# mmaker/c-lwe-snarks

Hardware: AMD Instinct MI355X
Metric: snark_proofs_per_sec (higher is better)
Workload: dtype u32 limbs (704-bit integers mod 2^704) + AES-256 bytes; int8 digits on the matrix cores, int32 accumulation (exact)

## Files before the change

c-lwe-snarks_amd/__init__.py:

```python
from __future__ import annotations

import ctypes
import os
from dataclasses import dataclass

import numpy as np

_HERE = os.path.dirname(os.path.abspath(__file__))
LIB_PATH = os.environ.get("MFHIP_LIB") or os.path.join(_HERE, "libmfhip.so")
P = 0xFFFFFFFB


class MfhError(RuntimeError):
    pass


@dataclass(frozen=True)
class Params:

    n: int = 1470
    logq: int = 736
    d: int = 1 << 15
    m: int = 21845

# ... 40 lines not shown

DEBUG = Params(d=256, m=64)
DEFAULT = Params()


class _CParams(ctypes.Structure):
    _fields_ = [("n", ctypes.c_uint32), ("logq", ctypes.c_uint32), ("d", ctypes.c_uint32), ("m", ctypes.c_uint32)]


_lib = None

EXPORTS = [
    "mfh_ctx_create", "mfh_ctx_destroy", "mfh_set_stream", "mfh_sync", "mfh_scrub_staging", "mfh_last_error", "mfh_set_seed",
    "mfh_keystream", "mfh_sample_rows", "mfh_ct_add", "mfh_ct_mul_ui", "mfh_ct_addmul_ui", "mfh_eval_rows",
    "mfh_encrypt_rows", "mfh_decrypt", "mfh_ct_smudge", "mfh_ssp_upload", "mfh_witness_poly", "mfh_version",
    "mfh_workspace_bytes", "mfh_last_kernel_ms", "mfh_set_timing", "mfh_set_overlap", "mfh_eval_rows_multi", "mfh_prove_batch", "mfh_crs_mm_image_bytes", "mfh_crs_expand_mm", "mfh_crs_set_resident_mm", "mfh_witness_poly_multi", "mfh_witness_poly_mm", "mfh_poly_h_multi", "mfh_poly_mul", "mfh_poly_add", "mfh_poly_prepare_t",
    "mfh_ssp_prepare", "mfh_poly_h", "mfh_setup_messages", "mfh_setup", "mfh_setup_image", "mfh_crs_image_set_b", "mfh_prove",
    "mfh_prove_partial", "mfh_prove_finish", "mfh_ct_to_lanes", "mfh_ct_from_lanes", "mfh_lanes_per_value", "mfh_digest128", "mfh_timing_drain", "mfh_timing_busy_ms", "mfh_timing_work_rows", "mfh_set_batch_image", "mfh_set_batch_slabs", "mfh_set_expand_path", "mfh_set_encrypt_path", "mfh_set_batch_launch", "mfh_set_batch_bw", "mfh_set_mm_chunk_rows", "mfh_set_mm_pack", "mfh_set_poly_exact", "mfh_poly_exact_fallbacks", "mfh_poly_exact_points", "mfh_set_poly_exact_points", "mfh_set_mm_stream", "mfh_add_dotp", "mfh_set_encrypt_chunks", "mfh_set_witness_per", "mfh_set_eval_path", "mfh_set_decrypt_path", "mfh_decrypt_rows",
    "mfh_crs_mm_share_bytes", "mfh_crs_expand_mm_share", "mfh_crs_set_resident_mm_share", "mfh_batch_chain", "mfh_batch_witness_cols", "mfh_batch_chain_from_w", "mfh_witness_poly_mm_cols", "mfh_prove_batch_partial", "mfh_prove_batch_finish",
    "mfh_resident_row_bytes", "mfh_crs_expand", "mfh_eval_rows_resident", "mfh_crs_set_resident",
    "mfh_witness_lanes", "mfh_witness_from_lanes", "mfh_prove_partial_w", "mfh_verify",
    "mfh_ssp_set_prg", "mfh_ssp_prg_make_t", "mfh_ssp_prg_fill",
    "mfh_resident_share_rows", "mfh_crs_expand_share", "mfh_crs_set_resident_share", "mfh_crs_set_resident_prefix",
    "mfh_prove_batch_supergroup", "mfh_prove_batch_stream_wait", "mfh_set_mm_width",
    "mfh_setup_public", "mfh_prove_public", "mfh_prove_batch_public", "mfh_vk_derive", "mfh_verify_public",
    "mfh_ssp_from_rows", "mfh_ssp_set_rows", "mfh_ssp_rows_fill", "mfh_ssp_rows_violations", "mfh_circuit_create", "mfh_circuit_destroy", "mfh_circuit_assign",
    "mfh_circuit_create_global", "mfh_circuit_create_ex", "mfh_circuit_create_out", "mfh_circuit_create_sum",
    "mfh_merkle_create", "mfh_merkle_destroy", "mfh_merkle_set_leaves", "mfh_merkle_root", "mfh_merkle_nodes", "mfh_merkle_paths",
    "mfh_sha256_records", "mfh_merkle_set_records", "mfh_merkle_update_rows", "mfh_merkle_update_records",
    "mfh_merkle_absent_rows", "mfh_merkle_insert_keys", "mfh_merkle_update_rows_cut", "mfh_merkle_update_records_cut", "mfh_merkle_insert_keys_cut",
    "mfh_merkle_remove_keys", "mfh_merkle_remove_keys_cut", "mfh_merkle_transfer_keys", "mfh_merkle_transfer_keys_cut",
    "mfh_merkle_paths_cut", "mfh_merkle_absent_rows_cut", "mfh_merkle_range_rows", "mfh_merkle_range_rows_cut",
]


def load_library():
    global _lib
    if _lib is not None:
        return _lib
    if not os.path.exists(LIB_PATH):
        raise MfhError(f"{LIB_PATH} is missing: run `python -c 'import __graft_entry__ as g; g.build()'` "
                       "(hipcc --offload-arch=gfx950).  There is no CPU fallback.")
    lib = ctypes.CDLL(LIB_PATH)
    vp, u64, sz, i32, u32 = ctypes.c_void_p, ctypes.c_uint64, ctypes.c_size_t, ctypes.c_int, ctypes.c_uint32
    sig = {
        "mfh_ctx_create": (i32, [ctypes.POINTER(vp), i32, ctypes.POINTER(_CParams)]),
        "mfh_ctx_destroy": (None, [vp]),
        "mfh_set_stream": (i32, [vp, vp]),
        "mfh_sync": (i32, [vp]),
        "mfh_scrub_staging": (i32, [vp]),
        "mfh_last_error": (ctypes.c_char_p, [vp]),
        "mfh_set_seed": (i32, [vp, ctypes.c_char_p]),
        "mfh_keystream": (i32, [vp, u64, vp, sz]),
        "mfh_sample_rows": (i32, [vp, u64, sz, vp]),
        "mfh_ct_add": (i32, [vp, vp, vp, vp, sz]),
        "mfh_ct_mul_ui": (i32, [vp, vp, vp, u32, sz]),
        "mfh_ct_addmul_ui": (i32, [vp, vp, vp, u32, sz]),
        "mfh_eval_rows": (i32, [vp, u64, sz, vp, vp, vp, vp, vp, i32]),
        "mfh_encrypt_rows": (i32, [vp, u64, sz, vp, vp, vp, vp]),
        "mfh_decrypt": (i32, [vp, vp, vp, sz, vp]),
        "mfh_ct_smudge": (i32, [vp, vp, sz, ctypes.c_char_p, sz, ctypes.c_char_p]),
        "mfh_ssp_upload": (i32, [vp, vp, vp, sz, sz]),
        "mfh_witness_poly": (i32, [vp, vp, ctypes.c_char_p, u32, vp]),
        "mfh_version": (ctypes.c_char_p, []),
        "mfh_workspace_bytes": (sz, [vp]),
        "mfh_last_kernel_ms": (ctypes.c_float, [vp, ctypes.c_char_p]),
        "mfh_set_timing": (i32, [vp, i32]),
        "mfh_set_overlap": (i32, [vp, i32]),
        "mfh_eval_rows_multi": (i32, [vp, u64, sz, vp, vp, u32, u32, vp, i32]),
        "mfh_poly_h_multi": (i32, [vp, vp, vp, u32]),
        "mfh_witness_poly_mm": (i32, [vp, vp, u32, ctypes.c_char_p, sz, vp, vp]),
        "mfh_witness_poly_multi": (i32, [vp, vp, u32, ctypes.c_char_p, sz, vp, vp]),
        "mfh_crs_mm_image_bytes": (sz, [vp]),
        "mfh_crs_expand_mm": (i32, [vp, vp, vp]),
        "mfh_crs_set_resident_mm": (i32, [vp, vp]),
        "mfh_prove_batch": (i32, [vp, vp, vp, u32, ctypes.c_char_p, sz, vp, ctypes.c_char_p, sz, ctypes.c_char_p, vp]),
        "mfh_prove_batch_supergroup": (u32, [vp]),
        "mfh_set_mm_width": (i32, [vp, u32, i32]),
        "mfh_prove_batch_stream_wait": (i32, [vp, u32, vp]),
        "mfh_poly_mul": (i32, [vp, vp, sz, vp, sz, vp]),
        "mfh_poly_add": (i32, [vp, vp, vp, sz, vp]),
        "mfh_poly_prepare_t": (i32, [vp, vp]),
        "mfh_ssp_prepare": (i32, [vp, vp]),
        "mfh_poly_h": (i32, [vp, vp, vp]),
        "mfh_setup_messages": (i32, [vp, vp, u32, u32, u32, vp]),
        "mfh_setup": (i32, [vp, vp, u32, u32, u32, vp, vp, vp]),
        "mfh_setup_image": (i32, [vp, vp, u32, u32, u32, vp, vp, vp, vp]),
        "mfh_prove": (i32, [vp, vp, vp, ctypes.c_char_p, u32, ctypes.c_char_p, sz, ctypes.c_char_p, vp]),
        "mfh_prove_partial": (i32, [vp, vp, vp, ctypes.c_char_p, u32, u32, u32, vp]),
        "mfh_prove_finish": (i32, [vp, vp, ctypes.c_char_p, sz, ctypes.c_char_p]),
        "mfh_lanes_per_value": (u32, [vp]),
        "mfh_digest128": (i32, [vp, vp, sz, vp]),
        "mfh_ct_to_lanes": (i32, [vp, vp, sz, vp]),
        "mfh_ct_from_lanes": (i32, [vp, vp, sz, vp]),
        "mfh_add_dotp": (i32, [vp, vp, vp, vp, sz]),
        "mfh_crs_set_resident_prefix": (i32, [vp, vp, sz]),
        "mfh_resident_share_rows": (sz, [vp, u32, u32]),
        "mfh_crs_expand_share": (i32, [vp, vp, u32, u32, vp]),
        "mfh_crs_set_resident_share": (i32, [vp, vp, u32, u32]),
        "mfh_ssp_set_prg": (i32, [vp, u64, vp]),
        "mfh_ssp_prg_make_t": (i32, [vp, u64, ctypes.c_char_p, vp]),
# ... 62 lines not shown
        "mfh_merkle_paths": (i32, [vp, vp, u32, vp, vp, sz]),
        "mfh_sha256_records": (i32, [vp, vp, sz, u32, u32, vp]),
        "mfh_merkle_set_records": (i32, [vp, vp, u32, u32, vp, sz, u32]),
        "mfh_merkle_update_rows": (i32, [vp, vp, u32, vp, vp, vp, sz, vp]),
        "mfh_merkle_update_records": (i32, [vp, vp, u32, vp, vp, sz, u32, vp, sz, vp, sz, vp]),
        "mfh_merkle_absent_rows": (i32, [vp, vp, vp, sz, u32, u32, u32, vp, sz, vp, sz, vp, vp]),
        "mfh_merkle_insert_keys": (i32, [vp, vp, vp, sz, u32, u32, u32, vp, sz, vp, sz, vp, sz, vp, vp, vp]),
        "mfh_merkle_update_rows_cut": (i32, [vp, vp, u32, vp, vp, u32, vp, vp, vp, vp]),
        "mfh_merkle_update_records_cut": (i32, [vp, vp, u32, vp, vp, sz, u32, vp, sz, u32, vp, vp, vp, vp]),
        "mfh_merkle_insert_keys_cut": (i32, [vp, vp, vp, sz, u32, u32, u32, vp, sz, vp, sz, u32, vp, vp, vp, vp, vp, vp]),
        "mfh_merkle_remove_keys": (i32, [vp, vp, vp, sz, u32, u32, u32, vp, sz, vp, sz, vp, vp, vp]),
        "mfh_merkle_remove_keys_cut": (i32, [vp, vp, vp, sz, u32, u32, u32, vp, sz, u32, vp, vp, vp, vp, vp, vp]),
        "mfh_merkle_transfer_keys": (i32, [vp, vp, vp, sz, u32, u32, u32, u32, vp, vp, sz, vp, vp, sz, vp, vp, vp]),
        "mfh_merkle_transfer_keys_cut": (i32, [vp, vp, vp, sz, u32, u32, u32, u32, vp, vp, sz, vp, u32, vp, vp, vp, vp, vp, vp]),
        "mfh_merkle_adjust_keys": (i32, [vp, vp, vp, sz, u32, u32, u32, u32, vp, sz, vp, vp, vp, sz, vp, vp, vp]),
        "mfh_merkle_adjust_keys_cut": (i32, [vp, vp, vp, sz, u32, u32, u32, u32, vp, sz, vp, vp, u32, vp, vp, vp, vp, vp, vp]),
        "mfh_merkle_balance_sum": (i32, [vp, vp, vp, sz, u32, u32, u32, vp, vp]),
        "mfh_merkle_paths_cut": (i32, [vp, vp, u32, vp, u32, vp, vp, vp]),
        "mfh_merkle_absent_rows_cut": (i32, [vp, vp, vp, sz, u32, u32, u32, vp, sz, u32, vp, vp, vp, vp, vp]),
        "mfh_merkle_range_rows": (i32, [vp, vp, vp, sz, u32, u32, vp, vp, u32, vp, vp, vp, vp, sz, vp]),
        "mfh_merkle_range_rows_cut": (i32, [vp, vp, vp, sz, u32, u32, vp, vp, u32, vp, vp, vp, u32, vp, vp, vp, vp]),
    }
    for name, (res, args) in sig.items():
        fn = getattr(lib, name)
        fn.restype = res
        fn.argtypes = args
    _lib = lib
    return lib


def rows_to_csr(rows):
    if isinstance(rows, tuple) and len(rows) == 3 and all(isinstance(a, np.ndarray) for a in rows):
        row_ptr, wire, coef = rows
    else:
        lens = [len(r) for r in rows]
        row_ptr = np.zeros(len(lens) + 1, dtype=np.int64)
        np.cumsum(lens, out=row_ptr[1:])
        flat = [(int(w), int(a) % P) for r in rows for (w, a) in r]
        wire = np.array([w for w, _ in flat], dtype=np.int64)
        coef = np.array([a for _, a in flat], dtype=np.int64)
    if len(row_ptr) == 0 or min(np.min(row_ptr), np.min(wire, initial=0), np.min(coef, initial=0)) < 0:
        raise MfhError("rows: row_ptr needs nrows + 1 entries, and no entry may be negative")
    if max(np.max(row_ptr), np.max(wire, initial=0), np.max(coef, initial=0)) > 0xFFFFFFFF:
        raise MfhError("rows: entries must fit 32 bits")
    return tuple(np.ascontiguousarray(a, dtype=np.uint32) for a in (row_ptr, wire, coef))

# ... 682 lines not shown
        self._chk(self.lib.mfh_set_encrypt_path(self._h, int(path)))

    def set_eval_path(self, path=0):
        self._chk(self.lib.mfh_set_eval_path(self._h, int(path)))

    def set_encrypt_chunks(self, chunks=0):
        self._chk(self.lib.mfh_set_encrypt_chunks(self._h, int(chunks)))

    def set_witness_per(self, statements=0):
        self._chk(self.lib.mfh_set_witness_per(self._h, int(statements)))

    def set_batch_launch(self, groups_per_launch=4, merge_regions=True):
        self._chk(self.lib.mfh_set_batch_launch(self._h, int(groups_per_launch), 1 if merge_regions else 0))

    def set_batch_bw(self, merged=True):
        self._chk(self.lib.mfh_set_batch_bw(self._h, 1 if merged else 0))

    def set_mm_stream(self, map=0, persistent=False, sync_mode=0, spin_max=64):
        self._chk(self.lib.mfh_set_mm_stream(self._h, int(map), int(persistent), int(sync_mode), int(spin_max)))

    def set_mm_width(self, per_xcd=32, early_chain=False):
        self._chk(self.lib.mfh_set_mm_width(self._h, int(per_xcd), 1 if early_chain else 0))

    def set_mm_pack(self, on=True):
        self._chk(self.lib.mfh_set_mm_pack(self._h, 1 if on else 0))

    def set_poly_exact(self, mode=1):
        self._chk(self.lib.mfh_set_poly_exact(self._h, int(mode)))

    def poly_exact_fallbacks(self):
        return int(self.lib.mfh_poly_exact_fallbacks(self._h))

    def exact_points(self):
        out = (ctypes.c_uint32 * 4)()
        self._chk(self.lib.mfh_poly_exact_points(self._h, out))
        return [int(x) for x in out]

    def set_exact_points(self, pts):
        if pts is None:
            self._chk(self.lib.mfh_set_poly_exact_points(self._h, None))
            return
        pts = [int(x) for x in pts]
        if len(pts) != 4 or not all(0 <= x < 2**32 for x in pts):
            raise MfhError(f"set_exact_points: four uint32 values, got {pts!r}")
        self._chk(self.lib.mfh_set_poly_exact_points(self._h, (ctypes.c_uint32 * 4)(*pts)))

# ... 490 lines not shown
```

c-lwe-snarks_amd/csrc/ctx.hpp:

```cpp
#pragma once
#include <hip/hip_runtime.h>

#include <stdint.h>
#include <string.h>

#include <string>
#include <vector>

#include "aes_dev.hpp"
#include "mfhip.h"
#include "ssp_prg.hpp"

#define HIP_TRY(ctx, expr)                                                        \
  do {                                                                            \
    hipError_t e_ = (expr);                                                       \
    if (e_ != hipSuccess) {                                                       \
      (ctx)->err = std::string(#expr) + ": " + hipGetErrorString(e_);             \
      return MFH_EDEVICE;                                                         \
    }                                                                             \
  } while (0)

struct PolyState;
struct SspInterp;
struct SspRows;
// ... 56 lines not shown
  DevBuf d_msg;
  DevBuf d_prover;
  std::vector<uint32_t> h_cw;
  const uint8_t *mm_image = nullptr;
  uint32_t mm_rank = 0, mm_world = 1;
  uint64_t mm_off[3] = {0, 0, 0}, mm_rows[3] = {0, 0, 0};
  size_t mm_base[3] = {0, 0, 0};
  DevBuf ssp_frag;
  const uint32_t *ssp_frag_src = nullptr;
  SspInterp *interp = nullptr;
  DevBuf circ_io;
  DevBuf circ_state;
  DevBuf d_batch;
  DevBuf batch_img;
  int batch_image = 1;
  int mm_map = 1;
  bool mm_persist = true;
  bool mm_wave1 = false;
  uint32_t mm_sync_mode = 0, mm_spin = 64;
  uint32_t mm_width = 32;
  size_t early_ws_half = 0;
  bool batch_early_chain = false;
  uint32_t *mm_sync = nullptr;
  int poly_exact = 1;
  bool poly_pts_pinned = false;
  uint32_t poly_pts[4] = {0, 0, 0, 0};
  bool mm_pack = true;
  uint32_t mm_chunk_rows = 131071;
  int expand_path = 0;
  int enc_path = 0;
  uint32_t ncu = 256;
  int dec_path = 0;
  int eval_path = 0;
  uint32_t enc_chunks = 0;
  uint32_t witness_per = 0;
  uint32_t batch_slabs = 0;
  int batch_bw_merged = 1;
  int batch_merge = 1;
  uint32_t batch_ngl = 8;
  PinBuf pin_rows, pin_cw, pin_smudge;
  PinBuf pin_pub;
  DevBuf d_pub;
  PinBuf pin_wring[8];
  uint32_t pin_wnext = 0;
  hipEvent_t ev_sample = nullptr;
  DevBuf sample_tmp;
// ... 188 lines not shown
```

c-lwe-snarks_amd/csrc/evalmm.hip:

```cpp
#include <algorithm>
#include <cstring>

#include "ctx.hpp"

namespace {

using mf::AesKey;

constexpr int CT = 4;
constexpr int SB = 88;
constexpr int VB = 92;
constexpr int MB = CT * SB;
constexpr int MT = MB / 32;
constexpr int RT = 128;
constexpr int TSTRIDE = 384;
constexpr int BLK_PER_ROW = 24;
static_assert(MB % 32 == 0 && CT * VB + 15 <= TSTRIDE, "tile geometry");

typedef int v4i __attribute__((ext_vector_type(4)));
typedef int v16i __attribute__((ext_vector_type(16)));

__device__ __forceinline__ uint32_t coef_at(const MmIo &io, uint32_t v, uint32_t nrows, uint32_t i) {
  if (io.bits) {
    const uint32_t a = io.bits_row0 + i;
    return a ? (io.bits[(uint64_t)v * io.bits_stride + ((a - 1) >> 3)] >> ((a - 1) & 7)) & 1u : 0u;
  }
// ... 444 lines not shown
  if (MODE == 0 && wave < MT2) {
    int *p = part + ((uint64_t)blockIdx.y * gridDim.x + blockIdx.x) * MB2 * N2;
#pragma unroll
    for (int q = 0; q < NQ2; q++)
#pragma unroll
      for (int e = 0; e < 4; e++) p[(uint64_t)(wave * 16 + 4 * g4 + e) * N2 + 16 * q + c16] = acc[q][e];
  }
}


#ifndef MMS_SW
#define MMS_SW 8
#endif
constexpr int SW = MMS_SW;
constexpr int TPW = 16;
#ifndef MMS_RQ
#define MMS_RQ 2
#endif
constexpr int RQ = MMS_RQ;
constexpr int RG = 16 / RQ;
constexpr int CG = SW / RG;
constexpr int CH = NQ2 / CG;
struct MmsImages { const v4i *image[16]; };
__device__ __forceinline__ void mms_item(uint32_t xcd, uint32_t slot, uint32_t ngt, uint32_t ngr, uint32_t map, uint32_t &grp, uint32_t &tg) {
  if (map == 0) {
    grp = slot % ngt;
    tg = (slot / ngt) * 8 + xcd;
  } else {
    const uint32_t blk = slot >> 5, i = slot & 31, nreg = ngt / ngr, tpb = 32 / ngr;
    grp = (blk % nreg) * ngr + i % ngr;
    tg = ((blk / nreg) * tpb + i / ngr) * 8 + xcd;
  }
}
__device__ __forceinline__ long long mms_pack_e(const v4i &a) {
  return (long long)a[0] + ((long long)a[1] << 8) + ((long long)a[2] << 16) + ((long long)a[3] << 24);
}
template <int CTRL>
__device__ __forceinline__ long long mms_quad_bcast(long long t) {
  const int lo = __builtin_amdgcn_update_dpp(0, (int)(unsigned int)(unsigned long long)t, CTRL, 0xf, 0xf, false);
  const int hi = __builtin_amdgcn_update_dpp(0, (int)((unsigned long long)t >> 32), CTRL, 0xf, 0xf, false);
  return (long long)(((unsigned long long)(unsigned int)hi << 32) | (unsigned int)lo);
}
__device__ __forceinline__ void mms_store_packed(int *__restrict__ part, uint32_t pk, uint64_t m4 , uint32_t ctile, uint32_t c16,
                                                 const v4i &acc) {
  const long long T = mms_pack_e(acc);
  if (pk == 1) {
    reinterpret_cast<long long *>(part)[m4 * N2 + 16 * ctile + c16] = T;
    return;
  }
  const long long T1 = mms_quad_bcast<0x55>(T), T2 = mms_quad_bcast<0xAA>(T), T3 = mms_quad_bcast<0xFF>(T);
  if (c16 & 3) return;
  const __int128 U = (__int128)T + (__int128)T1 * 256 + (__int128)T2 * 65536 + (__int128)T3 * 16777216;
  const unsigned __int128 u = (unsigned __int128)U;
  reinterpret_cast<uint4 *>(part)[m4 * (N2 / 4) + 4 * ctile + (c16 >> 2)] = uint4{(uint32_t)u, (uint32_t)(u >> 32), (uint32_t)(u >> 64), 0u};
}
__device__ __forceinline__ void mmstream_body(const MmsImages &imgs, uint32_t mtiles, uint32_t KS, uint32_t nrows, uint32_t rows_per_chunk,
// ... 131 lines not shown
  }
#pragma unroll
  for (int t = 0; t < RQ; t++) {
    if (mt0 + t >= mtiles) continue;
    int *p = part + ((uint64_t)chunk * Mtot + (uint64_t)(mt0 + t) * 16) * N2;
#pragma unroll
    for (int q = 0; q < CH; q++)
#pragma unroll
      for (int e = 0; e < 4; e++) p[(uint64_t)(4 * g4 + e) * N2 + 16 * (ch * CH + q) + c16] = acc[t][q][e];
  }
}

__global__ __launch_bounds__(SW * 64) void k_mmstream(MmsImages imgs, uint32_t mtiles, uint32_t KS, uint32_t nrows, uint32_t rows_per_chunk,
                                                      const v4i *__restrict__ cdv, int *__restrict__ part, uint32_t ngt, uint32_t ngr, uint32_t map,
                                                      uint64_t cd_stride, uint64_t part_stride, uint32_t pk) {
  uint32_t grp, tg;
  mms_item(blockIdx.x & 7, blockIdx.x >> 3, ngt, ngr, map, grp, tg);
  mmstream_body(imgs, mtiles, KS, nrows, rows_per_chunk, cdv, part, grp, tg, blockIdx.y, cd_stride, part_stride, pk);
}
__global__ __launch_bounds__(SW * 64) void k_mmstream1(MmsImages imgs, uint32_t mtiles, uint32_t KS, uint32_t nrows, uint32_t rows_per_chunk,
                                                       const v4i *__restrict__ cdv, int *__restrict__ part, uint32_t pk) {
  mmstream_body(imgs, mtiles, KS, nrows, rows_per_chunk, cdv, part, 0u, blockIdx.x, blockIdx.y, 0, 0, pk);
}
__device__ __forceinline__ void mmstream_persistent(const MmsImages &imgs, uint32_t mtiles, uint32_t KS, uint32_t nrows, uint32_t rows_per_chunk,
                                                    const v4i *__restrict__ cdv, int *__restrict__ part, uint32_t ngt, uint32_t ngr, uint32_t map,
                                                    uint64_t cd_stride, uint64_t part_stride, uint32_t nblk , uint32_t nchunks,
                                                    uint32_t *__restrict__ sync, uint32_t sync_mode, uint32_t spin_max, uint32_t width, uint32_t pk) {
  const uint32_t xcd = blockIdx.x & 7, cu = blockIdx.x >> 3;
  const uint32_t members = sync_mode == 2 ? 32u : (map ? ngr : ngt);
  uint32_t *ctr = sync + xcd * 32 + (sync_mode == 2 ? 0u : cu / members);
  uint32_t k = 0;
  for (uint32_t chunk = 0; chunk < nchunks; chunk++)
    for (uint32_t slot = cu; slot < nblk * 32; slot += width, k++) {
      if (sync_mode && members > 1) {
        if (threadIdx.x == 0) {
          __hip_atomic_fetch_add(ctr, 1u, __ATOMIC_RELAXED, __HIP_MEMORY_SCOPE_AGENT);
          const uint32_t target = (k + 1) * members;
          for (uint32_t spin = 0; spin < spin_max && __hip_atomic_load(ctr, __ATOMIC_RELAXED, __HIP_MEMORY_SCOPE_AGENT) < target; spin++) __builtin_amdgcn_s_sleep(8);
        }
        __syncthreads();
      }
      uint32_t grp, tg;
      mms_item(xcd, slot, ngt, ngr, map, grp, tg);
      mmstream_body(imgs, mtiles, KS, nrows, rows_per_chunk, cdv, part, grp, tg, chunk, cd_stride, part_stride, pk);
    }
}
__global__ __launch_bounds__(SW * 64) void k_mmstream_p(MmsImages imgs, uint32_t mtiles, uint32_t KS, uint32_t nrows, uint32_t rows_per_chunk,
                                                        const v4i *__restrict__ cdv, int *__restrict__ part, uint32_t ngt, uint32_t ngr, uint32_t map,
                                                        uint64_t cd_stride, uint64_t part_stride, uint32_t nblk, uint32_t nchunks,
                                                        uint32_t *__restrict__ sync, uint32_t sync_mode, uint32_t spin_max, uint32_t width, uint32_t pk) {
  mmstream_persistent(imgs, mtiles, KS, nrows, rows_per_chunk, cdv, part, ngt, ngr, map, cd_stride, part_stride, nblk, nchunks, sync, sync_mode, spin_max, width, pk);
}
__global__ __launch_bounds__(SW * 64) void k_mmstream_pb(MmsImages imgs, uint32_t mtiles, uint32_t KS, uint32_t nrows, uint32_t rows_per_chunk,
                                                         const v4i *__restrict__ cdv, int *__restrict__ part, uint32_t ngt, uint32_t ngr, uint32_t map,
                                                         uint64_t cd_stride, uint64_t part_stride, uint32_t nblk, uint32_t nchunks,
                                                         uint32_t *__restrict__ sync, uint32_t sync_mode, uint32_t spin_max, uint32_t width, uint32_t pk) {
  mmstream_persistent(imgs, mtiles, KS, nrows, rows_per_chunk, cdv, part, ngt, ngr, map, cd_stride, part_stride, nblk, nchunks, sync, sync_mode, spin_max, width, pk);
}

constexpr int WSW = 4, WRQ = 4;
__device__ __forceinline__ void mfma_acc(v4i &acc, const v4i &a, const v4i &b) {
  asm volatile("v_mfma_i32_16x16x64_i8 %0, %1, %2, %0" : "+a"(acc) : "v"(a), "v"(b));
}
__device__ __forceinline__ void mmstream_body_w(const MmsImages &imgs, uint32_t mtiles, uint32_t KS, uint32_t nrows, uint32_t rows_per_chunk,
                                                const v4i *__restrict__ cdv, int *__restrict__ part, uint32_t grp, uint32_t tg, uint32_t chunk, uint64_t cd_stride,
                                                uint64_t part_stride) {
  __shared__ v4i bfrag[2][RT2 / 64][NQ2][64];
  const uint32_t tid = threadIdx.x, lane = tid & 63;
  const uint32_t wave = __builtin_amdgcn_readfirstlane(tid >> 6);
  const uint32_t c16 = lane & 15, g4 = lane >> 4;
  if (tg * 16 >= mtiles) return;
  const v4i *__restrict__ image = imgs.image[grp];
  cdv += grp * cd_stride;
  part += grp * part_stride;
  const uint32_t mt0 = tg * 16 + wave * WRQ;
  const uint32_t r0 = chunk * rows_per_chunk, r1 = min(nrows, r0 + rows_per_chunk);
  if (r0 >= r1) return;
  constexpr int KSN = RT2 / 64;
  constexpr int BPK = NQ2 * 64 / (WSW * 64);
  v4i acc[WRQ][NQ2];
// ... 382 lines not shown
  if (mms_group_args(P, ios, nvecs, A)) {
    hipLaunchKernelGGL(k_mm_digits4w_groups, dim3((P.rpad / 16 + DG4 - 1) / DG4, P.ngt), dim3(256), 0, c->stream, A, P.nrows, P.rpad, P.cd, (uint64_t)P.cd_bytes);
    HIP_TRY(c, hipGetLastError());
    return MFH_OK;
  }
  for (uint32_t g = 0; g < P.ngt; g++) {
    if (P.ND == 4 && !ios[g].bits)
      hipLaunchKernelGGL(k_mm_digits4w, dim3((P.rpad / 16 + DG4 - 1) / DG4), dim3(256), 0, c->stream, ios[g], nvecs[g], P.nrows, P.rpad, P.cd + g * P.cd_bytes,
                         ios[g].sc_zeroed);
    else
      hipLaunchKernelGGL(k_mm_digits, dim3((P.rpad / 16 + DG_RG - 1) / DG_RG), dim3(N2), 0, c->stream, ios[g], nvecs[g], P.ND, P.nrows, P.rpad, (uint32_t)NQ2, 1,
                         P.cd + g * P.cd_bytes, ios[g].sc_zeroed);
  }
  HIP_TRY(c, hipGetLastError());
  return MFH_OK;
}
static bool mms_persistent(const mfh_ctx *c, const MmsPlan &P) {
  return P.ngt > 1 && c->mm_persist && c->ncu == 256 && ((c->mm_map && 32 % P.ng == 0) || 32 % P.ngt == 0);
}
static uint32_t mms_pk(const mfh_ctx *c, const MmsPlan &P) {
  if (!c->mm_pack || (mms_persistent(c, P) && c->mm_wave1)) return 0;
  return P.ND;
}
int mms_stream(mfh_ctx *c, const MmsPlan &P) {
  const uint32_t KS = (P.nrows + RT2 - 1) / RT2 * (RT2 / 64), tgs = (P.mtiles + TPW - 1) / TPW;
  const bool will_persist = mms_persistent(c, P);
  Timer t(c, P.ngt > 1 ? (P.ND == 1 ? 14 : 10) : 8, P.nrows, (uint64_t)P.nrows * P.ngt, will_persist ? 1 : 0);
  MmsImages imgs{};
  for (uint32_t g = 0; g < P.ngt; g++) imgs.image[g] = (const v4i *)P.img[g / P.ng];
  const uint32_t pk = mms_pk(c, P);
  if (P.ngt > 1) {
    const uint32_t tgx = (tgs + 7) / 8;
    const uint32_t map = c->mm_map && 32 % P.ng == 0 ? 1u : 0u;
    const uint32_t slots = map ? (tgx + 32 / P.ng - 1) / (32 / P.ng) * (P.ngt / P.ng) * 32 : tgx * P.ngt;
    const bool persistent = will_persist;
    if (persistent && c->mm_wave1) {
      hipLaunchKernelGGL(k_mmstream_w, dim3(256), dim3(WSW * 64), 0, c->stream, imgs, P.mtiles, KS, P.nrows, P.rpc, (const v4i *)P.cd, P.part, P.ngt, P.ng, map,
                         (uint64_t)(P.cd_bytes / 16), (uint64_t)(P.part_bytes / 4), (slots + 31) / 32, P.nchunks);
    } else if (persistent) {
      if (!c->mm_sync) HIP_TRY(c, hipMalloc(&c->mm_sync, 8 * 32 * sizeof(uint32_t)));
      if (c->mm_sync_mode) HIP_TRY(c, hipMemsetAsync(c->mm_sync, 0, 8 * 32 * sizeof(uint32_t), c->stream));
      const uint32_t width = P.ND == 1 ? 32u : c->mm_width;
      hipLaunchKernelGGL(P.ND == 1 ? k_mmstream_pb : k_mmstream_p, dim3(8 * width), dim3(SW * 64), 0, c->stream, imgs, P.mtiles, KS, P.nrows, P.rpc, (const v4i *)P.cd, P.part, P.ngt, P.ng, map,
                         (uint64_t)(P.cd_bytes / 16), (uint64_t)(P.part_bytes / 4), (slots + 31) / 32, P.nchunks, c->mm_sync, width == 32 ? c->mm_sync_mode : 0u, c->mm_spin, width, pk);
    } else {
      hipLaunchKernelGGL(k_mmstream, dim3(slots * 8, P.nchunks), dim3(SW * 64), 0, c->stream, imgs, P.mtiles, KS, P.nrows, P.rpc, (const v4i *)P.cd, P.part, P.ngt, P.ng,
                         map, (uint64_t)(P.cd_bytes / 16), (uint64_t)(P.part_bytes / 4), pk);
    }
  } else
    hipLaunchKernelGGL(k_mmstream1, dim3((tgs + 7) / 8 * 8, P.nchunks), dim3(SW * 64), 0, c->stream, imgs, P.mtiles, KS, P.nrows, P.rpc, (const v4i *)P.cd, P.part, pk);
  HIP_TRY(c, hipGetLastError());
  return MFH_OK;
}
int mms_finish(mfh_ctx *c, const MmsPlan &P, const MmIo *ios, const uint32_t *nvecs, int accumulate) {
  const WideGeom wg = wide_geom(c);
  const uint32_t n = c->P.n;
  const uint32_t pk = mms_pk(c, P);
  MmGroupArgs A;
  if (mms_group_args(P, ios, nvecs, A)) {
    uint32_t nvmax = 0;
    for (uint32_t g = 0; g < P.ngt; g++) nvmax = std::max(nvmax, nvecs[g]);
    FINISH_LAUNCH(k_evalmm_finish_groups, 4, pk, dim3(n + 1, (nvmax + 63) / 64, P.ngt), P.part, (uint64_t)(P.part_bytes / 4), P.nchunks, P.ntiles, (uint32_t)N2, n, P.nrows,
                  wg.ct, wg.mbp, wg.sby, wg.LL, A, accumulate);
    HIP_TRY(c, hipGetLastError());
    return MFH_OK;
  }
  for (uint32_t g = 0; g < P.ngt; g++) {
// ... 93 lines not shown
      hipLaunchKernelGGL((k_evalmm16<1, 1472>), grid, dim3(1024), 0, c->stream, keyx, c->d_t0, ctr_ct * sh.row0[r], n, (uint32_t)sh.rows[r], rpc, c8,
                         (const int8_t *)nullptr, (int *)nullptr, d_image + base);
    base += mm_region_bytes(c, sh.rows[r]);
  }
  HIP_TRY(c, hipGetLastError());
  return MFH_OK;
}
int mfh_crs_expand_mm(mfh_ctx *c, const uint8_t *d_crs_c8, uint8_t *d_image) { return mfh_crs_expand_mm_share(c, d_crs_c8, 0, 1, d_image); }
int mfh_set_mm_stream(mfh_ctx *c, int map, int persistent, int sync_mode, uint32_t spin_max) {
  if (!c || map < 0 || map > 1 || sync_mode < 0 || sync_mode > 2 || persistent < 0 || persistent > 2) return MFH_EINVAL;
  c->mm_map = map;
  c->mm_persist = persistent != 0;
  c->mm_wave1 = persistent == 2;
  c->mm_sync_mode = (uint32_t)sync_mode;
  c->mm_spin = spin_max;
  return MFH_OK;
}
int mfh_set_mm_width(mfh_ctx *c, uint32_t per_xcd, int early_chain) {
  if (!c || per_xcd < 1 || per_xcd > 32) return MFH_EINVAL;
  c->mm_width = per_xcd;
  c->batch_early_chain = early_chain != 0;
  return MFH_OK;
}
int mfh_set_mm_pack(mfh_ctx *c, int on) {
  if (!c) return MFH_EINVAL;
  c->mm_pack = on != 0;
  return MFH_OK;
}
int mfh_set_mm_chunk_rows(mfh_ctx *c, uint32_t rows) {
  if (!c || rows > 131071) return MFH_EINVAL;
  c->mm_chunk_rows = rows ? rows : 131071;
  return MFH_OK;
}
int mfh_crs_set_resident_mm_share(mfh_ctx *c, const uint8_t *d_image, uint32_t rank, uint32_t world) {
  if (!c || !world || rank >= world) return MFH_EINVAL;
  c->mm_image = d_image;
  c->mm_rank = rank;
  c->mm_world = world;
  const uint64_t ctr_ct = (uint64_t)wide_geom(c).vby * c->P.n;
  const MmShare sh = mm_share(c, rank, world);
  size_t base = 0;
  for (int r = 0; r < 3; r++) {
    c->mm_off[r] = ctr_ct * sh.row0[r];
    c->mm_rows[r] = sh.rows[r];
    c->mm_base[r] = base;
    base += mm_region_bytes(c, sh.rows[r]);
// ... 7 lines not shown
```

include/mfhip.h:

```cpp
#pragma once
#include <stddef.h>
#include <stdint.h>

#ifdef __cplusplus
extern "C" {
#endif

#define MFH_P 0xfffffffbu

enum {
  MFH_OK = 0,
  MFH_EINVAL = -1,
  MFH_EDEVICE = -2,
  MFH_ENOMEM = -3,
  MFH_EUNSUPPORTED = -4
};

typedef struct {
  uint32_t n;
  uint32_t logq;
  uint32_t d;
  uint32_t m;
} mfh_params;

// ... 173 lines not shown
                     const uint64_t *d_err, uint8_t *d_crs_c8, void *d_rows_image);
int mfh_prove_public(mfh_ctx *ctx, const uint8_t *d_crs_c8, const uint32_t *d_ssp, uint32_t lu, const uint8_t *h_bits, uint32_t delta,
                     const uint8_t *h_smudge_mag, size_t maglen, const uint8_t *h_smudge_sign, uint64_t *d_proof);
int mfh_prove_batch_public(mfh_ctx *ctx, const uint8_t *d_crs_c8, const uint32_t *d_ssp, uint32_t lu, uint32_t nproofs, const uint8_t *h_bits,
                           size_t bits_stride, const uint32_t *h_delta, const uint8_t *h_smudge_mag, size_t maglen, const uint8_t *h_smudge_sign,
                           uint64_t *d_proofs);
int mfh_vk_derive(mfh_ctx *ctx, const uint32_t *d_ssp, uint32_t s, uint32_t lu, uint32_t *d_vk);
int mfh_verify_public(mfh_ctx *ctx, const uint32_t *d_vk, uint32_t lu, uint32_t alpha, uint32_t beta, const uint64_t *d_sk, const uint64_t *d_proofs,
                      const uint8_t *h_statements, size_t stmt_stride, size_t count, uint8_t *d_ok);

size_t mfh_crs_mm_image_bytes(const mfh_ctx *ctx);
int mfh_crs_expand_mm(mfh_ctx *ctx, const uint8_t *d_crs_c8, uint8_t *d_image);
int mfh_crs_set_resident_mm(mfh_ctx *ctx, const uint8_t *d_image);
int mfh_set_expand_path(mfh_ctx *ctx, int path);
int mfh_set_batch_image(mfh_ctx *ctx, int enabled);
int mfh_set_batch_slabs(mfh_ctx *ctx, uint32_t nslabs);
int mfh_set_encrypt_chunks(mfh_ctx *ctx, uint32_t chunks);
int mfh_set_eval_path(mfh_ctx *ctx, int path);
int mfh_set_witness_per(mfh_ctx *ctx, uint32_t statements);
int mfh_set_batch_launch(mfh_ctx *ctx, uint32_t groups_per_launch, int merge_regions);
int mfh_set_batch_bw(mfh_ctx *ctx, int merged);
int mfh_set_mm_stream(mfh_ctx *ctx, int map, int persistent, int sync_mode, uint32_t spin_max);
int mfh_set_mm_width(mfh_ctx *ctx, uint32_t per_xcd, int early_chain);
int mfh_set_mm_chunk_rows(mfh_ctx *ctx, uint32_t rows);
int mfh_set_mm_pack(mfh_ctx *ctx, int on);
int mfh_prove_batch(mfh_ctx *ctx, const uint8_t *d_crs_c8, const uint32_t *d_ssp, uint32_t nproofs, const uint8_t *h_witness_bits,
                    size_t bits_stride, const uint32_t *h_delta, const uint8_t *h_smudge_mag, size_t maglen, const uint8_t *h_smudge_sign,
                    uint64_t *d_proofs);
uint32_t mfh_prove_batch_supergroup(const mfh_ctx *ctx);
int mfh_prove_batch_stream_wait(mfh_ctx *ctx, uint32_t upto, void *hip_stream);
size_t mfh_crs_mm_share_bytes(const mfh_ctx *ctx, uint32_t rank, uint32_t world);
int mfh_crs_expand_mm_share(mfh_ctx *ctx, const uint8_t *d_crs_c8, uint32_t rank, uint32_t world, uint8_t *d_image);
int mfh_crs_set_resident_mm_share(mfh_ctx *ctx, const uint8_t *d_image, uint32_t rank, uint32_t world);
int mfh_batch_chain(mfh_ctx *ctx, const uint32_t *d_ssp, uint32_t nstmt, const uint8_t *h_witness_bits, size_t bits_stride, const uint32_t *h_delta,
                    uint32_t *d_w, uint32_t *d_h, uint32_t *d_v);
int mfh_batch_witness_cols(mfh_ctx *ctx, const uint32_t *d_ssp, uint32_t nstmt, const uint8_t *h_witness_bits, size_t bits_stride, const uint32_t *h_delta,
                           uint32_t col0, uint32_t ncols, uint32_t *d_w, size_t w_stride);
int mfh_batch_chain_from_w(mfh_ctx *ctx, const uint32_t *d_ssp, uint32_t nstmt, const uint32_t *d_w, uint32_t *d_h, uint32_t *d_v);
int mfh_prove_batch_partial(mfh_ctx *ctx, const uint8_t *d_crs_c8, uint32_t rank, uint32_t world, uint32_t nstmt, const uint8_t *h_witness_bits,
                            size_t bits_stride, const uint32_t *d_w, const uint32_t *d_h, const uint32_t *d_v, size_t coef_stride, uint64_t *d_partial);
int mfh_prove_batch_finish(mfh_ctx *ctx, const uint8_t *d_crs_c8, uint32_t nstmt, const uint32_t *h_delta, const uint8_t *h_smudge_mag, size_t maglen,
                           const uint8_t *h_smudge_sign, uint64_t *d_proofs);

int mfh_prove_partial(mfh_ctx *ctx, const uint8_t *d_crs_c8, const uint32_t *d_ssp, const uint8_t *h_witness_bits, uint32_t delta,
                      uint32_t rank, uint32_t world, uint64_t *d_partial);
int mfh_prove_finish(mfh_ctx *ctx, uint64_t *d_proof, const uint8_t *h_smudge_mag, size_t maglen, const uint8_t *h_smudge_sign);
// ... 31 lines not shown
```

Before: 13460.

## Add atomic work-stealing queue to persistent matrix-stream kernel tail

```diff
diff --git a/c-lwe-snarks_amd/__init__.py b/c-lwe-snarks_amd/__init__.py
--- a/c-lwe-snarks_amd/__init__.py
+++ b/c-lwe-snarks_amd/__init__.py
@@ -86,7 +86,7 @@
     "mfh_witness_lanes", "mfh_witness_from_lanes", "mfh_prove_partial_w", "mfh_verify",
     "mfh_ssp_set_prg", "mfh_ssp_prg_make_t", "mfh_ssp_prg_fill",
     "mfh_resident_share_rows", "mfh_crs_expand_share", "mfh_crs_set_resident_share", "mfh_crs_set_resident_prefix",
-    "mfh_prove_batch_supergroup", "mfh_prove_batch_stream_wait", "mfh_set_mm_width",
+    "mfh_prove_batch_supergroup", "mfh_prove_batch_stream_wait", "mfh_set_mm_width", "mfh_set_mm_queue", "mfh_set_mm_claim_log", "mfh_mm_claim_log_launches",
     "mfh_setup_public", "mfh_prove_public", "mfh_prove_batch_public", "mfh_vk_derive", "mfh_verify_public",
     "mfh_ssp_from_rows", "mfh_ssp_set_rows", "mfh_ssp_rows_fill", "mfh_ssp_rows_violations", "mfh_circuit_create", "mfh_circuit_destroy", "mfh_circuit_assign",
     "mfh_circuit_create_global", "mfh_circuit_create_ex", "mfh_circuit_create_out", "mfh_circuit_create_sum",
@@ -96,6 +96,13 @@
     "mfh_merkle_remove_keys", "mfh_merkle_remove_keys_cut", "mfh_merkle_transfer_keys", "mfh_merkle_transfer_keys_cut",
     "mfh_merkle_paths_cut", "mfh_merkle_absent_rows_cut", "mfh_merkle_range_rows", "mfh_merkle_range_rows_cut",
 ]
+
+
+OPTIONAL_EXPORTS = {
+    "mfh_set_mm_queue": "tuning knob; older builds walk fixed lists",
+    "mfh_set_mm_claim_log": "test instrumentation of mfh_set_mm_queue",
+    "mfh_mm_claim_log_launches": "test instrumentation of mfh_set_mm_queue",
+}
 
 
 def load_library():
@@ -141,6 +148,9 @@
         "mfh_prove_batch": (i32, [vp, vp, vp, u32, ctypes.c_char_p, sz, vp, ctypes.c_char_p, sz, ctypes.c_char_p, vp]),
         "mfh_prove_batch_supergroup": (u32, [vp]),
         "mfh_set_mm_width": (i32, [vp, u32, i32]),
+        "mfh_set_mm_queue": (i32, [vp, i32, u32, i32]),
+        "mfh_set_mm_claim_log": (i32, [vp, vp, sz]),
+        "mfh_mm_claim_log_launches": (u32, [vp, ctypes.POINTER(u32), u32]),
         "mfh_prove_batch_stream_wait": (i32, [vp, u32, vp]),
         "mfh_poly_mul": (i32, [vp, vp, sz, vp, sz, vp]),
         "mfh_poly_add": (i32, [vp, vp, vp, sz, vp]),
@@ -249,6 +259,8 @@
         "mfh_merkle_range_rows_cut": (i32, [vp, vp, vp, sz, u32, u32, vp, vp, u32, vp, vp, vp, u32, vp, vp, vp, vp]),
     }
     for name, (res, args) in sig.items():
+        if name in OPTIONAL_EXPORTS and not hasattr(lib, name):
+            continue
         fn = getattr(lib, name)
         fn.restype = res
         fn.argtypes = args
@@ -977,6 +989,21 @@
     def set_mm_width(self, per_xcd=32, early_chain=False):
         self._chk(self.lib.mfh_set_mm_width(self._h, int(per_xcd), 1 if early_chain else 0))
 
+    def set_mm_queue(self, mode=1, start_shift=0, prefix=-8):
+        self._chk(self.lib.mfh_set_mm_queue(self._h, int(mode), int(start_shift), int(prefix)))
+
+    def set_mm_claim_log(self, log):
+        if log is None:
+            self._chk(self.lib.mfh_set_mm_claim_log(self._h, None, 0))
+        else:
+            self._chk(self.lib.mfh_set_mm_claim_log(self._h, log.data_ptr(), log.numel()))
+
+    def mm_claim_log_launches(self):
+        out = (ctypes.c_uint32 * (16 * 12))()
+        n = int(self.lib.mfh_mm_claim_log_launches(self._h, out, 16))
+        keys = ("offset", "nchunks", "nblk", "ngt", "ngr", "map", "tgs", "width", "coeff_bytes", "queue", "prefix", "shift")
+        return [dict(zip(keys, (int(x) for x in out[12 * i:12 * i + 12]))) for i in range(n)]
+
     def set_mm_pack(self, on=True):
         self._chk(self.lib.mfh_set_mm_pack(self._h, 1 if on else 0))
 
diff --git a/c-lwe-snarks_amd/csrc/ctx.hpp b/c-lwe-snarks_amd/csrc/ctx.hpp
--- a/c-lwe-snarks_amd/csrc/ctx.hpp
+++ b/c-lwe-snarks_amd/csrc/ctx.hpp
@@ -102,6 +102,8 @@
   size_t early_ws_half = 0;
   bool batch_early_chain = false;
   uint32_t *mm_sync = nullptr;
+  uint32_t mm_queue = 1, mm_queue_shift = 0; int mm_queue_prefix = -8;
+  uint32_t *mm_log = nullptr; size_t mm_log_words = 0, mm_log_used = 0; uint32_t mm_log_n = 0, mm_log_desc[16][12];
   int poly_exact = 1;
   bool poly_pts_pinned = false;
   uint32_t poly_pts[4] = {0, 0, 0, 0};
diff --git a/c-lwe-snarks_amd/csrc/evalmm.hip b/c-lwe-snarks_amd/csrc/evalmm.hip
--- a/c-lwe-snarks_amd/csrc/evalmm.hip
+++ b/c-lwe-snarks_amd/csrc/evalmm.hip
@@ -2,6 +2,7 @@
 #include <cstring>
 
 #include "ctx.hpp"
+#include "mms_slots.hpp"
 
 namespace {
 
@@ -492,16 +493,6 @@
 constexpr int CG = SW / RG;
 constexpr int CH = NQ2 / CG;
 struct MmsImages { const v4i *image[16]; };
-__device__ __forceinline__ void mms_item(uint32_t xcd, uint32_t slot, uint32_t ngt, uint32_t ngr, uint32_t map, uint32_t &grp, uint32_t &tg) {
-  if (map == 0) {
-    grp = slot % ngt;
-    tg = (slot / ngt) * 8 + xcd;
-  } else {
-    const uint32_t blk = slot >> 5, i = slot & 31, nreg = ngt / ngr, tpb = 32 / ngr;
-    grp = (blk % nreg) * ngr + i % ngr;
-    tg = ((blk / nreg) * tpb + i / ngr) * 8 + xcd;
-  }
-}
 __device__ __forceinline__ long long mms_pack_e(const v4i &a) {
   return (long long)a[0] + ((long long)a[1] << 8) + ((long long)a[2] << 16) + ((long long)a[3] << 24);
 }
@@ -679,16 +670,44 @@
                                                        const v4i *__restrict__ cdv, int *__restrict__ part, uint32_t pk) {
   mmstream_body(imgs, mtiles, KS, nrows, rows_per_chunk, cdv, part, 0u, blockIdx.x, blockIdx.y, 0, 0, pk);
 }
+struct MmsQueue {
+  uint32_t *ctr;
+  uint32_t *log;
+  uint32_t mode, shift, prefix, tgs;
+};
+#ifdef MMS_ITEM_STAMPS
+#define MMS_STAMP_PARAM , unsigned long long *__restrict__ stamps
+#define MMS_STAMP_ARG , stamps
+#else
+#define MMS_STAMP_PARAM
+#define MMS_STAMP_ARG
+#endif
 __device__ __forceinline__ void mmstream_persistent(const MmsImages &imgs, uint32_t mtiles, uint32_t KS, uint32_t nrows, uint32_t rows_per_chunk,
                                                     const v4i *__restrict__ cdv, int *__restrict__ part, uint32_t ngt, uint32_t ngr, uint32_t map,
                                                     uint64_t cd_stride, uint64_t part_stride, uint32_t nblk , uint32_t nchunks,
-                                                    uint32_t *__restrict__ sync, uint32_t sync_mode, uint32_t spin_max, uint32_t width, uint32_t pk) {
+                                                    uint32_t *__restrict__ sync, uint32_t sync_mode, uint32_t spin_max, uint32_t width, uint32_t pk,
+                                                    const MmsQueue &q MMS_STAMP_PARAM) {
+  __shared__ uint32_t claim[2];
   const uint32_t xcd = blockIdx.x & 7, cu = blockIdx.x >> 3;
   const uint32_t members = sync_mode == 2 ? 32u : (map ? ngr : ngt);
   uint32_t *ctr = sync + xcd * 32 + (sync_mode == 2 ? 0u : cu / members);
-  uint32_t k = 0;
-  for (uint32_t chunk = 0; chunk < nchunks; chunk++)
-    for (uint32_t slot = cu; slot < nblk * 32; slot += width, k++) {
+  const uint32_t per_chunk = nblk * 32, total = nchunks * per_chunk;
+  uint32_t k = 0, chunk = 0, slot = cu;
+  uint32_t qi = 0;
+#ifdef MMS_ITEM_STAMPS
+  unsigned long long t_first = 0, t_left = 0;
+  uint32_t items = 0, foreign = 0;
+#endif
+  for (;;) {
+#ifdef MMS_ITEM_STAMPS
+    if (threadIdx.x == 0) t_left = __builtin_amdgcn_s_memrealtime();
+#endif
+    uint32_t ixcd = xcd, ichunk, islot, from = 0xffu;
+    if (chunk < nchunks && (!q.mode || k < q.prefix)) {
+      ichunk = chunk;
+      islot = slot;
+      slot += width;
+      if (slot >= per_chunk) slot = cu, chunk++;
       if (sync_mode && members > 1) {
         if (threadIdx.x == 0) {
           __hip_atomic_fetch_add(ctr, 1u, __ATOMIC_RELAXED, __HIP_MEMORY_SCOPE_AGENT);
@@ -697,22 +716,74 @@
         }
         __syncthreads();
       }
-      uint32_t grp, tg;
-      mms_item(xcd, slot, ngt, ngr, map, grp, tg);
-      mmstream_body(imgs, mtiles, KS, nrows, rows_per_chunk, cdv, part, grp, tg, chunk, cd_stride, part_stride, pk);
-    }
+      k++;
+    } else if (q.mode) {
+      if (threadIdx.x == 0) {
+        uint32_t flat = total;
+        while (qi < 8) {
+          const uint32_t qx = (xcd + q.shift + qi) & 7;
+          const uint32_t n = q.prefix * width + __hip_atomic_fetch_add(q.ctr + qx, 1u, __ATOMIC_RELAXED, __HIP_MEMORY_SCOPE_AGENT);
+          if (n >= total) {
+            qi++;
+          } else if (mms_slot_valid(qx, n % per_chunk, ngt, ngr, map, q.tgs)) {
+            flat = n;
+            break;
+          }
+        }
+        claim[0] = flat;
+        claim[1] = qi;
+      }
+      __syncthreads();
+      const uint32_t flat = __builtin_amdgcn_readfirstlane(claim[0]);
+      from = __builtin_amdgcn_readfirstlane(claim[1]);
+      __syncthreads();
+      if (flat >= total) break;
+      ixcd = (xcd + q.shift + from) & 7;
+      mms_flat(flat, nblk, ichunk, islot);
+    } else
+      break;
+    if (q.log && threadIdx.x == 0 && mms_slot_valid(ixcd, islot, ngt, ngr, map, q.tgs)) {
+      uint32_t *e = q.log + 2 * ((uint64_t)(ichunk * 8 + ixcd) * per_chunk + islot);
+      __hip_atomic_fetch_add(e, 1u, __ATOMIC_RELAXED, __HIP_MEMORY_SCOPE_AGENT);
+      e[1] = (blockIdx.x + 1) | (from << 16);
+    }
+#ifdef MMS_ITEM_STAMPS
+    if (threadIdx.x == 0 && mms_slot_valid(ixcd, islot, ngt, ngr, map, q.tgs)) {
+      if (!items) t_first = t_left;
+      items++;
+      foreign += ixcd != xcd;
+    }
+#endif
+    uint32_t grp, tg;
+    mms_item(ixcd, islot, ngt, ngr, map, grp, tg);
+    mmstream_body(imgs, mtiles, KS, nrows, rows_per_chunk, cdv, part, grp, tg, ichunk, cd_stride, part_stride, pk);
+  }
+#ifdef MMS_ITEM_STAMPS
+  if (threadIdx.x == 0) {
+    asm volatile("s_waitcnt vmcnt(0)" ::: "memory");
+    unsigned long long *st = stamps + 4 * (uint64_t)blockIdx.x;
+    st[0] = t_first;
+    st[1] = t_left;
+    st[2] = __builtin_amdgcn_s_memrealtime();
+    st[3] = items | ((unsigned long long)foreign << 32);
+  }
+#endif
 }
 __global__ __launch_bounds__(SW * 64) void k_mmstream_p(MmsImages imgs, uint32_t mtiles, uint32_t KS, uint32_t nrows, uint32_t rows_per_chunk,
                                                         const v4i *__restrict__ cdv, int *__restrict__ part, uint32_t ngt, uint32_t ngr, uint32_t map,
                                                         uint64_t cd_stride, uint64_t part_stride, uint32_t nblk, uint32_t nchunks,
-                                                        uint32_t *__restrict__ sync, uint32_t sync_mode, uint32_t spin_max, uint32_t width, uint32_t pk) {
-  mmstream_persistent(imgs, mtiles, KS, nrows, rows_per_chunk, cdv, part, ngt, ngr, map, cd_stride, part_stride, nblk, nchunks, sync, sync_mode, spin_max, width, pk);
+                                                        uint32_t *__restrict__ sync, uint32_t sync_mode, uint32_t spin_max, uint32_t width, uint32_t pk,
+                                                        MmsQueue q MMS_STAMP_PARAM) {
+  mmstream_persistent(imgs, mtiles, KS, nrows, rows_per_chunk, cdv, part, ngt, ngr, map, cd_stride, part_stride, nblk, nchunks, sync, sync_mode, spin_max, width, pk,
+                      q MMS_STAMP_ARG);
 }
 __global__ __launch_bounds__(SW * 64) void k_mmstream_pb(MmsImages imgs, uint32_t mtiles, uint32_t KS, uint32_t nrows, uint32_t rows_per_chunk,
                                                          const v4i *__restrict__ cdv, int *__restrict__ part, uint32_t ngt, uint32_t ngr, uint32_t map,
                                                          uint64_t cd_stride, uint64_t part_stride, uint32_t nblk, uint32_t nchunks,
-                                                         uint32_t *__restrict__ sync, uint32_t sync_mode, uint32_t spin_max, uint32_t width, uint32_t pk) {
-  mmstream_persistent(imgs, mtiles, KS, nrows, rows_per_chunk, cdv, part, ngt, ngr, map, cd_stride, part_stride, nblk, nchunks, sync, sync_mode, spin_max, width, pk);
+                                                         uint32_t *__restrict__ sync, uint32_t sync_mode, uint32_t spin_max, uint32_t width, uint32_t pk,
+                                                         MmsQueue q MMS_STAMP_PARAM) {
+  mmstream_persistent(imgs, mtiles, KS, nrows, rows_per_chunk, cdv, part, ngt, ngr, map, cd_stride, part_stride, nblk, nchunks, sync, sync_mode, spin_max, width, pk,
+                      q MMS_STAMP_ARG);
 }
 
 constexpr int WSW = 4, WRQ = 4;
@@ -1141,6 +1212,16 @@
   if (!c->mm_pack || (mms_persistent(c, P) && c->mm_wave1)) return 0;
   return P.ND;
 }
+#ifdef MMS_ITEM_STAMPS
+static unsigned long long *g_mms_stamps = nullptr;
+static uint32_t g_mms_stamp_n = 0, g_mms_stamp_kind[64];
+static unsigned long long *mms_stamps_next(uint32_t nd, uint32_t queue) {
+  if (!g_mms_stamps && hipMalloc(&g_mms_stamps, 64 * 256 * 4 * sizeof(unsigned long long)) != hipSuccess) return nullptr;
+  if (g_mms_stamp_n == 64) return nullptr;
+  g_mms_stamp_kind[g_mms_stamp_n] = nd | queue << 8;
+  return g_mms_stamps + (size_t)g_mms_stamp_n++ * 256 * 4;
+}
+#endif
 int mms_stream(mfh_ctx *c, const MmsPlan &P) {
   const uint32_t KS = (P.nrows + RT2 - 1) / RT2 * (RT2 / 64), tgs = (P.mtiles + TPW - 1) / TPW;
   const bool will_persist = mms_persistent(c, P);
@@ -1149,19 +1230,39 @@
   for (uint32_t g = 0; g < P.ngt; g++) imgs.image[g] = (const v4i *)P.img[g / P.ng];
   const uint32_t pk = mms_pk(c, P);
   if (P.ngt > 1) {
-    const uint32_t tgx = (tgs + 7) / 8;
     const uint32_t map = c->mm_map && 32 % P.ng == 0 ? 1u : 0u;
-    const uint32_t slots = map ? (tgx + 32 / P.ng - 1) / (32 / P.ng) * (P.ngt / P.ng) * 32 : tgx * P.ngt;
+    const uint32_t slots = mms_slots(tgs, P.ngt, P.ng, map);
     const bool persistent = will_persist;
     if (persistent && c->mm_wave1) {
       hipLaunchKernelGGL(k_mmstream_w, dim3(256), dim3(WSW * 64), 0, c->stream, imgs, P.mtiles, KS, P.nrows, P.rpc, (const v4i *)P.cd, P.part, P.ngt, P.ng, map,
                          (uint64_t)(P.cd_bytes / 16), (uint64_t)(P.part_bytes / 4), (slots + 31) / 32, P.nchunks);
     } else if (persistent) {
-      if (!c->mm_sync) HIP_TRY(c, hipMalloc(&c->mm_sync, 8 * 32 * sizeof(uint32_t)));
-      if (c->mm_sync_mode) HIP_TRY(c, hipMemsetAsync(c->mm_sync, 0, 8 * 32 * sizeof(uint32_t), c->stream));
+      constexpr size_t SYNC_WORDS = 8 * 32 + 2 * 8;
+      if (!c->mm_sync) HIP_TRY(c, hipMalloc(&c->mm_sync, SYNC_WORDS * sizeof(uint32_t)));
       const uint32_t width = P.ND == 1 ? 32u : c->mm_width;
+      const uint32_t sync_mode = width == 32 ? c->mm_sync_mode : 0u, nblk = (slots + 31) / 32;
+      uint32_t *qctr = c->mm_sync + 8 * 32 + 8 * (c->mm_ws_sel ? 1 : 0);
+      MmsQueue q{qctr, nullptr, c->mm_queue && !sync_mode ? 1u : 0u, c->mm_queue_shift & 7, 0u, tgs};
+      if (q.mode && !q.shift && nblk * 32 % width == 0) {
+        const uint32_t rounds = P.nchunks * (nblk * 32 / width);
+        q.prefix = c->mm_queue_prefix < 0 ? rounds - std::min(rounds, (uint32_t)-(int64_t)c->mm_queue_prefix) : std::min(rounds, (uint32_t)c->mm_queue_prefix);
+      }
+      if (sync_mode) HIP_TRY(c, hipMemsetAsync(c->mm_sync, 0, 8 * 32 * sizeof(uint32_t), c->stream));
+      else if (q.mode) HIP_TRY(c, hipMemsetAsync(qctr, 0, 8 * sizeof(uint32_t), c->stream));
+      if (c->mm_log) {
+        const size_t need = (size_t)2 * P.nchunks * 8 * nblk * 32;
+        if (c->mm_log_n == 16 || c->mm_log_used + need > c->mm_log_words) { c->err = "mfh_set_mm_claim_log: the log is too small for the call's launches"; return MFH_EINVAL; }
+        q.log = c->mm_log + c->mm_log_used;
+        const uint32_t desc[12] = {(uint32_t)c->mm_log_used, P.nchunks, nblk, P.ngt, P.ng, map, tgs, width, P.ND, q.mode, q.prefix, q.shift};
+        memcpy(c->mm_log_desc[c->mm_log_n++], desc, sizeof(desc));
+        c->mm_log_used += need;
+      }
+#ifdef MMS_ITEM_STAMPS
+      unsigned long long *stamps = mms_stamps_next(P.ND, q.mode);
+      if (!stamps) { c->err = "MMS_ITEM_STAMPS: no room for another launch"; return MFH_EINVAL; }
+#endif
       hipLaunchKernelGGL(P.ND == 1 ? k_mmstream_pb : k_mmstream_p, dim3(8 * width), dim3(SW * 64), 0, c->stream, imgs, P.mtiles, KS, P.nrows, P.rpc, (const v4i *)P.cd, P.part, P.ngt, P.ng, map,
-                         (uint64_t)(P.cd_bytes / 16), (uint64_t)(P.part_bytes / 4), (slots + 31) / 32, P.nchunks, c->mm_sync, width == 32 ? c->mm_sync_mode : 0u, c->mm_spin, width, pk);
+                         (uint64_t)(P.cd_bytes / 16), (uint64_t)(P.part_bytes / 4), nblk, P.nchunks, c->mm_sync, sync_mode, c->mm_spin, width, pk, q MMS_STAMP_ARG);
     } else {
       hipLaunchKernelGGL(k_mmstream, dim3(slots * 8, P.nchunks), dim3(SW * 64), 0, c->stream, imgs, P.mtiles, KS, P.nrows, P.rpc, (const v4i *)P.cd, P.part, P.ngt, P.ng,
                          map, (uint64_t)(P.cd_bytes / 16), (uint64_t)(P.part_bytes / 4), pk);
@@ -1301,6 +1402,40 @@
   c->batch_early_chain = early_chain != 0;
   return MFH_OK;
 }
+int mfh_set_mm_queue(mfh_ctx *c, int mode, uint32_t start_shift, int prefix) {
+  if (!c || mode < 0 || mode > 1 || start_shift > 7) return MFH_EINVAL;
+  c->mm_queue = (uint32_t)mode;
+  c->mm_queue_shift = start_shift;
+  c->mm_queue_prefix = prefix;
+  return MFH_OK;
+}
+int mfh_set_mm_claim_log(mfh_ctx *c, uint32_t *d_log, size_t words) {
+  if (!c || (d_log && !words)) return MFH_EINVAL;
+  c->mm_log = d_log;
+  c->mm_log_words = d_log ? words : 0;
+  c->mm_log_used = 0;
+  c->mm_log_n = 0;
+  return MFH_OK;
+}
+uint32_t mfh_mm_claim_log_launches(const mfh_ctx *c, uint32_t *desc, uint32_t max_launches) {
+  if (!c) return 0;
+  const uint32_t n = std::min(c->mm_log_n, max_launches);
+  if (desc && n) memcpy(desc, c->mm_log_desc, (size_t)n * 12 * sizeof(uint32_t));
+  return c->mm_log_n;
+}
+#ifdef MMS_ITEM_STAMPS
+uint32_t mfh_mm_item_stamps(unsigned long long *h_out, uint32_t max_launches) {
+  const uint32_t n = std::min(g_mms_stamp_n, max_launches);
+  if (hipDeviceSynchronize() != hipSuccess) return 0;
+  for (uint32_t l = 0; l < n; l++) {
+    unsigned long long *o = h_out + (size_t)l * 257 * 4;
+    o[0] = g_mms_stamp_kind[l], o[1] = o[2] = o[3] = 0;
+    if (hipMemcpy(o + 4, g_mms_stamps + (size_t)l * 256 * 4, 256 * 4 * sizeof(unsigned long long), hipMemcpyDeviceToHost) != hipSuccess) return 0;
+  }
+  g_mms_stamp_n = 0;
+  return n;
+}
+#endif
 int mfh_set_mm_pack(mfh_ctx *c, int on) {
   if (!c) return MFH_EINVAL;
   c->mm_pack = on != 0;
diff --git a/c-lwe-snarks_amd/csrc/mms_slots.hpp b/c-lwe-snarks_amd/csrc/mms_slots.hpp
--- /dev/null
+++ b/c-lwe-snarks_amd/csrc/mms_slots.hpp
@@ -0,0 +1,33 @@
+#pragma once
+#include <stdint.h>
+
+#if defined(__HIPCC__)
+#define MMS_HD __host__ __device__ __forceinline__
+#else
+#define MMS_HD inline
+#endif
+
+MMS_HD void mms_item(uint32_t xcd, uint32_t slot, uint32_t ngt, uint32_t ngr, uint32_t map, uint32_t &grp, uint32_t &tg) {
+  if (map == 0) {
+    grp = slot % ngt;
+    tg = (slot / ngt) * 8 + xcd;
+  } else {
+    const uint32_t blk = slot >> 5, i = slot & 31, nreg = ngt / ngr, tpb = 32 / ngr;
+    grp = (blk % nreg) * ngr + i % ngr;
+    tg = ((blk / nreg) * tpb + i / ngr) * 8 + xcd;
+  }
+}
+MMS_HD uint32_t mms_slots(uint32_t tgs, uint32_t ngt, uint32_t ngr, uint32_t map) {
+  const uint32_t tgx = (tgs + 7) / 8;
+  return map ? (tgx + 32 / ngr - 1) / (32 / ngr) * (ngt / ngr) * 32 : tgx * ngt;
+}
+MMS_HD uint32_t mms_nblk(uint32_t tgs, uint32_t ngt, uint32_t ngr, uint32_t map) { return (mms_slots(tgs, ngt, ngr, map) + 31) / 32; }
+MMS_HD bool mms_slot_valid(uint32_t xcd, uint32_t slot, uint32_t ngt, uint32_t ngr, uint32_t map, uint32_t tgs) {
+  uint32_t grp, tg;
+  mms_item(xcd, slot, ngt, ngr, map, grp, tg);
+  return tg < tgs;
+}
+MMS_HD void mms_flat(uint32_t flat, uint32_t nblk, uint32_t &chunk, uint32_t &slot) {
+  chunk = flat / (nblk * 32);
+  slot = flat % (nblk * 32);
+}
diff --git a/include/mfhip.h b/include/mfhip.h
--- a/include/mfhip.h
+++ b/include/mfhip.h
@@ -219,6 +219,9 @@
 int mfh_set_batch_bw(mfh_ctx *ctx, int merged);
 int mfh_set_mm_stream(mfh_ctx *ctx, int map, int persistent, int sync_mode, uint32_t spin_max);
 int mfh_set_mm_width(mfh_ctx *ctx, uint32_t per_xcd, int early_chain);
+int mfh_set_mm_queue(mfh_ctx *ctx, int mode, uint32_t start_shift, int prefix);
+int mfh_set_mm_claim_log(mfh_ctx *ctx, uint32_t *d_log, size_t words);
+uint32_t mfh_mm_claim_log_launches(const mfh_ctx *ctx, uint32_t *desc, uint32_t max_launches);
 int mfh_set_mm_chunk_rows(mfh_ctx *ctx, uint32_t rows);
 int mfh_set_mm_pack(mfh_ctx *ctx, int on);
 int mfh_prove_batch(mfh_ctx *ctx, const uint8_t *d_crs_c8, const uint32_t *d_ssp, uint32_t nproofs, const uint8_t *h_witness_bits,
```

After: 13970 (median of 6 runs). 3.8% higher.
